# UCSD-Comp-Imaging/Nerf-Simple

Hardware: AMD Instinct MI355X
Metric: ray-samples/sec at 800x800x128 (higher is better)
Workload: dtype f16

## Files before the change

nerf-simple_amd/csrc/mlp_bf16_16.hip:

```cpp
#include "composite_device.h"
#include "launchers.h"

using namespace nerf_layout;

#ifdef NERF_HALF
typedef _Float16 elem_t;
#define NERF_MFMA __builtin_amdgcn_mfma_f32_16x16x32_f16
#define NERF_KERNEL nerf_mlp_f16_16_kernel
#define NERF_LAUNCH nerf_amd_launch_mlp_f16_16
#else
typedef __bf16 elem_t;
#define NERF_MFMA __builtin_amdgcn_mfma_f32_16x16x32_bf16
#define NERF_KERNEL nerf_mlp_bf16_16_kernel
#define NERF_LAUNCH nerf_amd_launch_mlp_bf16_16
#endif
#include "mlp16_chain.h"

namespace {

#ifdef NERF_HALF
constexpr bool FOLD = true;
#else
constexpr bool FOLD = false;
#endif
struct MlpPlan {
    static constexpr int LAYERS = NUM_LAYERS;
    static constexpr bool SAVE = !FOLD;
    static constexpr int tpc(int L) { return L == 0 ? 8 : 4; }
    static constexpr int mt(int L) { return FOLD ? fold_mt(L) : b16_mt(L); }
    static constexpr int layer_off_kib(int L) { return FOLD ? fold_layer_off_kib(L) : b16_layer_off_kib(L); }
    static constexpr int bias_off(int L) { return FOLD ? fold_bias_off(L) : b16_bias_off(L); }
};
static_assert(NUM_CHUNKS<MlpPlan> == (FOLD ? 34 : 38) && plan_fits<MlpPlan>(), "chunks per tile / weight buffer, parity");

constexpr int LDS_POSD = LDS_CHAIN_END;
constexpr int LDS_POSX = LDS_POSD + WAVES * NCB * 1024;
constexpr int LDS_TOTAL = LDS_POSX + WAVES * NCB * 2048;
constexpr int RING_PTS = 1024;
constexpr int LDS_RING_RAW = LDS_TOTAL;
constexpr int LDS_RING_T = LDS_RING_RAW + RING_PTS * 16;
constexpr int LDS_TOTAL_COMP = LDS_RING_T + RING_PTS * 4;
constexpr int COMP_MAX_N = RING_PTS - TILE_PTS;
static_assert(COMP_MAX_N == FUSED_RENDER_MAX_N, "api.hip routes by this limit");
static_assert(LDS_TOTAL_COMP <= 160 * 1024, "LDS budget");
static_assert((RING_PTS & (RING_PTS - 1)) == 0 && RING_PTS % TILE_PTS == 0, "ring indexing");

static_assert(ACT_TILE_PTS == TILE_PTS && MASK_TILE_PTS == TILE_PTS, "activation blocks and mask tiles are the kernel's tiles");

struct State {
    using Plan = MlpPlan;
    ex8 X[NCB][8], Y[NCB][8];
    f32x4 pend[NCB][2];
    float sigma[NCB], rgb[NCB][3];
    bool bad;
    unsigned posd_off[NCB];
    char* acts;
    long long P;
    long long tile;
    int loff[NCB];
    unsigned mb[NCB][2];
    float amax[4];
    long long mask_tile;
    long long p_end;
    unsigned ring_q0;
    WFrag* wf;
};

template <bool RAYS, int SAVE, bool COMP>
__device__ __forceinline__ void stage_inputs(const Ctx& c, const MlpArgs& a, long long tile_base, State& st) {
    const int col = c.lane & 15, g = c.lane >> 4;
    float u_mine = 0.f;
    bool dev_rng = false;
    long long b0 = 0;
    int r0 = 0;
    if constexpr (RAYS) {
        b0 = tile_base / a.N;
        r0 = (int)(tile_base - b0 * a.N);
    }
    const long long p_end = COMP ? st.p_end : a.P;
    const int last_local = (int)(p_end - 1 - tile_base);
    constexpr bool RAY_POSD = RAYS && !SAVE;
    if constexpr (RAY_POSD) {
        const int top = last_local < TILE_PTS - 1 ? last_local : TILE_PTS - 1;
        const int nrays = (int)(split_point(b0, r0, top, a.N).b - b0) + 1;
        for (int idx = threadIdx.x; idx < nrays * 32; idx += WAVES * 64) {
            const int ray = idx >> 5, slot = idx & 31, gg = slot >> 3, sl = slot & 7;
            const float* rp = a.rays + (b0 + ray) * 6 + 3;
            const float dx = rp[0], dy = rp[1], dz = rp[2];
            const float nrm = norm3(dx, dy, dz);
            float val = 0.f;
            if (sl < 6) {
                const int cd = sl >> 1;
                const float dc = __fdiv_rn(cd == 0 ? dx : cd == 1 ? dy : dz, nrm);
                val = enc_lane(to_revolutions(dc), 2 * gg + (sl & 1));
            } else if (sl == 6 && gg < 3) {
                val = __fdiv_rn(gg == 0 ? dx : gg == 1 ? dy : dz, nrm);
            }
            lds_store<elem_t>(LDS_POSD + ray * 64 + slot * 2, 0, (elem_t)val);
        }
    }
    if constexpr (RAYS && NCB == 2) {
        dev_rng = (a.flags & NERF_FLAG_DEVICE_RNG) && !(a.flags & NERF_FLAG_TS_GIVEN);
        if (dev_rng) {
            int lm = c.wave * 32 + (c.lane & 31);
            if (lm > last_local) lm = last_local;
            u_mine = device_rng_uniform(a, split_point(b0, r0, lm, a.N));
        }
    }
#pragma unroll
    for (int cb = 0; cb < NCB; ++cb) {
        long long p = tile_base + c.wave * (16 * NCB) + cb * 16 + col;
        const bool valid = p < p_end;
        st.loff[cb] = valid ? block_lane_offset(g, c.wave * (16 * NCB) + cb * 16 + col) : LOFF_INVALID;
        if constexpr (SAVE == 2) {
            if (cb == 0)
                st.loff[0] = tile_base + c.wave * 32 + 16 * (c.lane >> 5) + col < p_end ? f8_lane_offset(c.lane, c.wave) : LOFF_INVALID;
        }
        if (!valid) p = p_end - 1;
        PointIn pt;
        st.posd_off[cb] = c.b_posd + cb * 1024;
        if constexpr (RAYS) {
            const float u_cb = (NCB == 2) ? __shfl(u_mine, cb * 16 + col) : 0.f;
            int lp = c.wave * (16 * NCB) + cb * 16 + col;
            if (lp > last_local) lp = last_local;
            if (SAVE && a.pts) {
                pt = fetch_point_pts(a, p);
            } else {
                const RaySample rs = split_point(b0, r0, lp, a.N);
                if constexpr (RAY_POSD) st.posd_off[cb] = LDS_POSD + (unsigned)(rs.b - b0) * 64 + g * 16;
                pt = fetch_point_rays<!RAY_POSD>(a, p, rs, u_cb, dev_rng);
                if constexpr (COMP) {
                    if (valid && g == 0)
                        lds_store<float>(((st.ring_q0 + c.wave * (16 * NCB) + cb * 16 + col) & (RING_PTS - 1)) * 4, LDS_RING_T, pt.t);
                }
                if (valid && g == 0 && a.ts_out) a.ts_out[p] = pt.t;
            }
        } else {
            pt = fetch_point_pts(a, p);
        }
        {
            const float xyz[3] = {pt.x, pt.y, pt.z};
            float v[16];
#pragma unroll
            for (int cd = 0; cd < 3; ++cd) {
                const TwoF q = to_revolutions(xyz[cd]);
#pragma unroll
                for (int jj = 0; jj < 5; ++jj) v[cd * 5 + jj] = enc_lane(q, 5 * g + jj);
            }
            v[15] = g == 0 ? pt.x : g == 1 ? pt.y : g == 2 ? pt.z : 0.f;
#pragma unroll
            for (int e = 0; e < 2; ++e) {
                u32x4 r;
#pragma unroll
                for (int i = 0; i < 4; ++i) r[i] = pack2<false>(v[8 * e + 2 * i], v[8 * e + 2 * i + 1]);
                lds_store<u32x4>(c.b_posx, cb * 2048 + e * 1024, r);
            }
        }
        if constexpr (!RAY_POSD) {
            const float dd[3] = {pt.d1, pt.d2, pt.d3};
            float v[8];
#pragma unroll
            for (int cd = 0; cd < 3; ++cd) {
                const TwoF q = to_revolutions(dd[cd]);
#pragma unroll
                for (int jj = 0; jj < 2; ++jj) v[cd * 2 + jj] = enc_lane(q, 2 * g + jj);
            }
            v[6] = g == 0 ? pt.d1 : g == 1 ? pt.d2 : g == 2 ? pt.d3 : 0.f;
            v[7] = 0.f;
            u32x4 r;
#pragma unroll
            for (int i = 0; i < 4; ++i) r[i] = pack2<false>(v[2 * i], v[2 * i + 1]);
            lds_store<u32x4>(c.b_posd, cb * 1024, r);
        }
    }
}

template <bool RAYS, int SAVE, bool COMP>
__device__ __forceinline__ void run_tile(const Ctx& c, const MlpArgs& a, long long tile_base, State& st) {
    stage_inputs<RAYS, SAVE, COMP>(c, a, tile_base, st);
    run_layer<0, SAVE>(c, st, st.X, st.X);
    run_layer<1, SAVE>(c, st, st.X, st.Y);
    run_layer<2, SAVE>(c, st, st.Y, st.X);
    run_layer<3, SAVE>(c, st, st.X, st.Y);
    run_layer<4, SAVE>(c, st, st.Y, st.X);
    run_layer<5, SAVE>(c, st, st.X, st.Y);
    run_layer<6, SAVE>(c, st, st.Y, st.X);
    run_layer<7, SAVE>(c, st, st.X, st.Y);
    ex8 (&c_in)[NCB][8] = FOLD ? st.Y : st.X;
    ex8 (&c_out)[NCB][8] = FOLD ? st.X : st.Y;
    run_layer<8, SAVE>(c, st, st.Y, st.X);
    run_layer<9, SAVE>(c, st, c_in, c_out);
    run_layer<10, SAVE>(c, st, c_out, c_in);
    epilogue_piece<10, 0>(0, st.pend, st.X, st);
    for (int cb_ = 1; cb_ < NCB; ++cb_) epilogue_piece<10, 0>(4 * cb_, st.pend, st.X, st);
}

__device__ __forceinline__ bool finite4(float x, float y, float z, float w) {
    return __builtin_fabsf(x) + __builtin_fabsf(y) + __builtin_fabsf(z) + __builtin_fabsf(w) < __builtin_inff();
}

struct RingSamples {
    unsigned q0;
    __device__ __forceinline__ float t(int i) const {
        return lds_load<float>(((q0 + (unsigned)i) & (RING_PTS - 1)) * 4, LDS_RING_T);
    }
    __device__ __forceinline__ f32x4 c(int i) const {
        return lds_load<f32x4>(((q0 + (unsigned)i) & (RING_PTS - 1)) * 16, LDS_RING_RAW);
    }
};

template <bool RAYS, int SAVE, bool COMP>
__device__ __forceinline__ void kernel_body(const MlpArgs& a, long long ntiles) {
    static_assert(!COMP || (RAYS && !SAVE), "the fused render is the rays-mode inference kernel");
    using P = MlpPlan;
    Ctx c;
    c.wave = __builtin_amdgcn_readfirstlane(threadIdx.x >> 6);
    c.lane = threadIdx.x & 63;
    const char* img = reinterpret_cast<const char*>(a.packed);
    c.wrsrc = __builtin_amdgcn_make_buffer_rsrc(const_cast<char*>(img), 0, (int)B16_IMAGE_BYTES, 0x00020000);
    c.wave_goff = c.wave * 1024;
    c.lane16 = c.lane * 16;
#pragma unroll
    for (int p = 0; p < 2; ++p) {
        c.b_wread[p] = LDS_W0 + p * LDS_WBUF + c.lane * 16;
        c.s_wdst[p] = LDS_W0 + p * LDS_WBUF + c.wave * 1024;
    }
    c.b_bias = (c.lane >> 4) * 16;
    c.b_posx = LDS_POSX + c.wave * (NCB * 2048) + c.lane * 16;
    c.b_posd = LDS_POSD + c.wave * (NCB * 1024) + c.lane * 16;

    {
        const float* bsrc = reinterpret_cast<const float*>(img + (long long)B16_WEIGHT_KIB * 1024);
        for (int i = threadIdx.x; i < B16_BIAS_FLOATS; i += WAVES * 64)
            lds_store<float>(i * 4, LDS_BIAS, bsrc[i]);
        Stage<P, NUM_CHUNKS<P> - 1>::issue(c);
    }
    asm volatile("s_waitcnt vmcnt(0)" ::: "memory");
    __syncthreads();
    WFrag wf;
    {
        constexpr int F0 = chunk_tiles<P>(0) * (layer_desc(0).chain_k / 32 + layer_desc(0).extra_slots / 32);
#pragma unroll
        for (int f = 0; f < 4 && f < F0; ++f) wf.a[f] = lds_load<ex8>(c.b_wread[0], f * 1024);
        wf.bias0 = lds_load<f32x4>(c.b_bias, LDS_BIAS + P::bias_off(0) * 4);
    }

    if constexpr (!COMP) {
        for (long long tile = blockIdx.x; tile < ntiles; tile += gridDim.x) {
            const long long tile_base = tile * TILE_PTS;
            asm volatile("" : "+s"(c.wave_goff));
            State st;
            st.wf = &wf;
            st.acts = reinterpret_cast<char*>(a.acts);
            st.P = a.P;
            st.mask_tile = SAVE == 2 ? f8_mask_offset_bytes(0, tile, 0, a.P) : mask_offset_bytes(0, tile, 0, a.P);
            st.tile = tile;
            st.bad = false;
            run_tile<RAYS, SAVE, false>(c, a, tile_base, st);
            bool bad = st.bad;
            if (c.lane < 16) {
#pragma unroll
                for (int cb = 0; cb < NCB; ++cb) {
                    const long long p = tile_base + c.wave * (16 * NCB) + cb * 16 + c.lane;
                    if (p < a.P) {
                        const f32x4 o = {st.rgb[cb][0], st.rgb[cb][1], st.rgb[cb][2], st.sigma[cb]};
                        *reinterpret_cast<f32x4*>(a.raw + p * 4) = o;
                        bad |= !finite4(o[0], o[1], o[2], o[3]);
                    }
                }
            }
            flag_nonfinite(c, bad);
        }
    } else {
        const long long B = a.P / a.N;
        const long long r_lo = (long long)blockIdx.x * B / gridDim.x, r_hi = ((long long)blockIdx.x + 1) * B / gridDim.x;
        const long long range_base = r_lo * a.N;
        const int n_pts = (int)((r_hi - r_lo) * a.N);
        const nerf_composite::RayOut out{a.rgb, a.disp, a.alpha, a.acc, a.w, a.pixels};
        int next_ray = 0, n_complete = 0;
        for (int q_tile = 0; q_tile < n_pts; q_tile += TILE_PTS) {
            const long long tile_base = range_base + q_tile;
            asm volatile("" : "+s"(c.wave_goff));
            State st;
            st.wf = &wf;
            st.acts = nullptr;
            st.P = a.P;
            st.mask_tile = 0;
            st.tile = 0;
            st.p_end = range_base + n_pts;
            st.ring_q0 = (unsigned)q_tile & (RING_PTS - 1);
            st.bad = false;
            run_tile<true, false, true>(c, a, tile_base, st);
            bool bad = st.bad;
            if (c.lane < 16) {
#pragma unroll
                for (int cb = 0; cb < NCB; ++cb) {
                    const int local = c.wave * (16 * NCB) + cb * 16 + c.lane;
                    if (q_tile + local < n_pts) {
                        const f32x4 o = {st.rgb[cb][0], st.rgb[cb][1], st.rgb[cb][2], st.sigma[cb]};
                        lds_store<f32x4>(((st.ring_q0 + local) & (RING_PTS - 1)) * 16, LDS_RING_RAW, o);
                        bad |= !finite4(o[0], o[1], o[2], o[3]);
                    }
                }
            }
            flag_nonfinite(c, bad);
            asm volatile("s_waitcnt lgkmcnt(0)" ::: "memory");
            __builtin_amdgcn_s_barrier();
            asm volatile("" ::: "memory");
            const int done_q = q_tile + TILE_PTS < n_pts ? q_tile + TILE_PTS : n_pts;
            while ((n_complete + 1) * a.N <= done_q) ++n_complete;
            if (n_complete - next_ray >= WAVES || done_q + TILE_PTS - next_ray * a.N > RING_PTS || done_q == n_pts) {
                for (int ray = next_ray + c.wave; ray < n_complete; ray += WAVES) {
                    const long long gray = r_lo + ray;
                    const float* d = a.rays + gray * 6 + 3;
                    const float dnorm = nerf_composite::unit_dir_norm(d[0], d[1], d[2], true);
                    const RingSamples src{(unsigned)(ray * a.N) & (RING_PTS - 1)};
                    nerf_composite::composite_ray(src, a.N, c.lane, dnorm, gray, out);
                }
                next_ray = n_complete;
                asm volatile("s_waitcnt lgkmcnt(0)" ::: "memory");
                __builtin_amdgcn_s_barrier();
                asm volatile("" ::: "memory");
            }
        }
    }
}

template <bool RAYS, bool SAVE, bool COMP>
__global__ __launch_bounds__(WAVES * 64, WAVES / 4) void NERF_KERNEL(MlpArgs a, long long ntiles) {
    extern __shared__ __attribute__((aligned(16))) char smem[];
    (void)smem;
    kernel_body<RAYS, SAVE ? 1 : 0, COMP>(a, ntiles);
}
#ifndef NERF_HALF
__global__ __launch_bounds__(WAVES * 64, WAVES / 4) void nerf_mlp_train_e4m3_kernel(MlpArgs a, long long ntiles) {
    extern __shared__ __attribute__((aligned(16))) char smem[];
    (void)smem;
    kernel_body<true, 2, false>(a, ntiles);
}
#endif

}

extern "C" int NERF_LAUNCH(const MlpArgs* args, int rays_mode, hipStream_t stream) {
    (void)hipGetLastError();
    MlpArgs a = *args;
    if (a.P <= 0) return 0;
    const long long ntiles = (a.P + TILE_PTS - 1) / TILE_PTS;
    const int cus = device_cus();
    const long long grid = ntiles < cus ? ntiles : cus;
    hipError_t e = hipSuccess;
    const bool comp = a.rgb || a.disp || a.acc || a.alpha || a.w || a.pixels;
    if (comp) {
        if (!rays_mode || a.acts || a.N > COMP_MAX_N || a.P / grid + a.N >= (1ll << 31)) return -2;
        auto kern = NERF_KERNEL<true, false, true>;
        e = allow_dynamic_lds(reinterpret_cast<const void*>(kern), LDS_TOTAL_COMP);
        if (e != hipSuccess) return (int)e;
        hipLaunchKernelGGL(kern, dim3((unsigned)grid), dim3(WAVES * 64), LDS_TOTAL_COMP, stream, a, ntiles);
        return (int)hipGetLastError();
    }
#ifdef NERF_HALF
    if (a.acts) return -2;
    auto kern = rays_mode ? NERF_KERNEL<true, false, false> : NERF_KERNEL<false, false, false>;
#else
    if (a.acts && !rays_mode) return -2;
    if ((a.flags & NERF_FLAG_STORE_E4M3) && !a.acts) return -2;
    auto kern = a.acts ? ((a.flags & NERF_FLAG_STORE_E4M3) ? nerf_mlp_train_e4m3_kernel : NERF_KERNEL<true, true, false>)
                       : (rays_mode ? NERF_KERNEL<true, false, false> : NERF_KERNEL<false, false, false>);
#endif
    e = allow_dynamic_lds(reinterpret_cast<const void*>(kern), LDS_TOTAL);
    if (e != hipSuccess) return (int)e;
    hipLaunchKernelGGL(kern, dim3((unsigned)grid), dim3(WAVES * 64), LDS_TOTAL, stream, a, ntiles);
    return (int)hipGetLastError();
}
```

nerf-simple_amd/csrc/nerf_device.h:

```cpp
#pragma once
#include <hip/hip_runtime.h>
#include <stdint.h>
#include <atomic>
#include "nerf_layout.h"

typedef __bf16 bf16x8 __attribute__((ext_vector_type(8)));
typedef __bf16 bf16x2 __attribute__((ext_vector_type(2)));
typedef short s16x2 __attribute__((ext_vector_type(2)));
typedef unsigned short u16x2 __attribute__((ext_vector_type(2)));
typedef float f32x2 __attribute__((ext_vector_type(2)));
typedef float f32x4 __attribute__((ext_vector_type(4)));
typedef float f32x16 __attribute__((ext_vector_type(16)));
typedef unsigned u32x4 __attribute__((ext_vector_type(4)));

#define NERF_FLAG_TS_GIVEN 1u
#define NERF_FLAG_DEVICE_RNG 2u
#define NERF_FLAG_SEED_IN_MEMORY 4u
#define NERF_FLAG_STORE_E4M3 8u

struct MlpArgs {
    const float* pts;
    const float* rays;
    const float* u;
    const float* tbins;
    const void* packed;
    float* raw;
    float* ts_out;
    void* acts;
    long long P;
    long long ray_id0;
    unsigned long long seed;
    int N;
    unsigned flags;
    float* rgb;
    float* disp;
    float* alpha;
    float* acc;
    float* w;
    float* pixels;
};

struct DensityArgs {
    const float* pts;
    long long stride;
    const void* packed;
    float* sigma;
    long long P;
    long long ny, nz;
    float lo[3], step[3];
};

constexpr int NERF_MAX_DEVICES = 64;
inline int device_cus() {
    static int cache[NERF_MAX_DEVICES] = {};
    int dev = 0;
    if (hipGetDevice(&dev) != hipSuccess || dev < 0 || dev >= NERF_MAX_DEVICES) return 256;
    if (cache[dev] == 0) {
        int cus = 256;
        if (hipDeviceGetAttribute(&cus, hipDeviceAttributeMultiprocessorCount, dev) != hipSuccess || cus <= 0) cus = 256;
        cache[dev] = cus;
    }
    return cache[dev];
}
inline hipError_t allow_dynamic_lds(const void* kernel, int bytes) {
    struct Slot { const void* kernel; int dev; };
    static Slot slots[128];
    static std::atomic<int> used{0};
    int dev = 0;
    if (hipGetDevice(&dev) != hipSuccess) dev = -1;
    const int n = used.load(std::memory_order_acquire);
    for (int i = 0; i < n && i < 128; ++i)
        if (slots[i].kernel == kernel && slots[i].dev == dev) return hipSuccess;
    const hipError_t e = hipFuncSetAttribute(kernel, hipFuncAttributeMaxDynamicSharedMemorySize, bytes);
    if (e == hipSuccess && dev >= 0) {
        const int i = used.load(std::memory_order_relaxed);
        if (i < 128) {
            slots[i] = Slot{kernel, dev};
            used.store(i + 1, std::memory_order_release);
        }
    }
    return e;
}

constexpr int LOFF_INVALID = 0x40000000;
__host__ __device__ constexpr int swapped_chunk(int g) { return (g & 1) * 2 + (g >> 1); }
__host__ __device__ constexpr int block_lane_offset(int g, int local) { return swapped_chunk(g) * 4096 + local * 16; }

template <int AUX = 0>
__device__ __forceinline__ void store_granule(__amdgpu_buffer_rsrc_t rs, int voffset, int soffset, u32x4 w) {
    const auto s0 = __builtin_amdgcn_permlane16_swap(w[0], w[2], false, false);
    const auto s1 = __builtin_amdgcn_permlane16_swap(w[1], w[3], false, false);
    const unsigned o0 = s0[0], o1 = s1[0], o2 = s0[1], o3 = s1[1];
    __builtin_amdgcn_raw_buffer_store_b128(u32x4{o0, o1, o2, o3}, rs, voffset, soffset, AUX);
    asm volatile("s_nop 1" ::"v"(o0), "v"(o1), "v"(o2), "v"(o3) : "memory");
}

template <bool ABS>
__device__ __forceinline__ float f8_absmax(float running, float v0, float v1) {
    float r;
    if constexpr (ABS) asm("v_max3_f32 %0, %1, |%2|, |%3|" : "=v"(r) : "v"(running), "v"(v0), "v"(v1));
    else asm("v_max3_f32 %0, %1, %2, %3" : "=v"(r) : "v"(running), "v"(v0), "v"(v1));
    return r;
}
__device__ __forceinline__ int f8_wave_max_exponent(float m) {
    int r;
    asm volatile("s_nop 1\n\t"
                 "v_max_f32_dpp %1, %1, %1 quad_perm:[1,0,3,2] row_mask:0xf bank_mask:0xf\n\ts_nop 1\n\t"
                 "v_max_f32_dpp %1, %1, %1 quad_perm:[2,3,0,1] row_mask:0xf bank_mask:0xf\n\ts_nop 1\n\t"
                 "v_max_f32_dpp %1, %1, %1 row_half_mirror row_mask:0xf bank_mask:0xf\n\ts_nop 1\n\t"
                 "v_max_f32_dpp %1, %1, %1 row_mirror row_mask:0xf bank_mask:0xf\n\ts_nop 1\n\t"
                 "v_max_f32_dpp %1, %1, %1 row_bcast:15 row_mask:0xa bank_mask:0xf\n\ts_nop 1\n\t"
                 "v_max_f32_dpp %1, %1, %1 row_bcast:31 row_mask:0xc bank_mask:0xf\n\ts_nop 1\n\t"
                 "v_readlane_b32 %0, %1, 63"
                 : "=s"(r), "+v"(m));
    return (r >> 23) & 0xff;
}
__device__ __forceinline__ unsigned f8_cvt4(unsigned lo, unsigned hi, float scale) {
    unsigned r;
    asm("v_cvt_scalef32_pk_fp8_bf16 %0, %1, %3\n\tv_cvt_scalef32_pk_fp8_bf16 %0, %2, %3 op_sel:[0,0,1]"
        : "=&v"(r) : "v"(lo), "v"(hi), "s"(scale));
    return r;
}
__host__ __device__ constexpr int f8_lane_offset(int lane, int wave) {
    return ((lane >> 4) & 1) * 4096 + (wave * 32 + 16 * (lane >> 5) + (lane & 15)) * 16;
}
template <int AUX = 0>
__device__ __forceinline__ void store_fragment_f8(__amdgpu_buffer_rsrc_t rs_data, int voff, int soff_data, u32x4 w0, u32x4 w1,
                                                  float scale) {
    const unsigned a0 = f8_cvt4(w0[0], w0[1], scale), b0 = f8_cvt4(w0[2], w0[3], scale);
    unsigned a1 = f8_cvt4(w1[0], w1[1], scale), b1 = f8_cvt4(w1[2], w1[3], scale);
    asm volatile("s_nop 1" : "+v"(a1), "+v"(b1));
    const auto x0 = __builtin_amdgcn_permlane32_swap(a0, a1, false, false);
    const auto x1 = __builtin_amdgcn_permlane32_swap(b0, b1, false, false);
    const auto y0 = __builtin_amdgcn_permlane16_swap(x0[0], x1[0], false, false);
    const auto y1 = __builtin_amdgcn_permlane16_swap(x0[1], x1[1], false, false);
    const unsigned o0 = y0[0], o1 = y0[1], o2 = y1[0], o3 = y1[1];
#if defined(F8_TIMING) && F8_TIMING == 2
    asm volatile("" ::"v"(o0), "v"(o1), "v"(o2), "v"(o3));
#else
    __builtin_amdgcn_raw_buffer_store_b128(u32x4{o0, o1, o2, o3}, rs_data, voff, soff_data,
#if defined(F8_TIMING) && F8_TIMING == 3
                                           0);
#else
                                           AUX);
#endif
    asm volatile("s_nop 1" ::"v"(o0), "v"(o1), "v"(o2), "v"(o3) : "memory");
#endif
}
constexpr int F8_GROUP = 4;
template <int AUX = 0>
__device__ __forceinline__ void store_group_f8(__amdgpu_buffer_rsrc_t rs_data, int voff, int soff_data,
                                               __amdgpu_buffer_rsrc_t rs_scale, int lane, int scale_byte,
                                               const u32x4 (&w0)[F8_GROUP], const u32x4 (&w1)[F8_GROUP], float amax) {
#if defined(F8_TIMING) && F8_TIMING == 1
    const int e = (__builtin_bit_cast(int, amax) >> 23) & 0xff;
#else
    const int e = f8_wave_max_exponent(amax);
#endif
    const int sb = e > 8 ? e - 7 : 1;
    const float scale = __builtin_bit_cast(float, sb << 23);
#pragma unroll
    for (int k = 0; k < F8_GROUP; ++k) store_fragment_f8<AUX>(rs_data, voff, soff_data + k * 8192, w0[k], w1[k], scale);
#if !(defined(F8_TIMING) && F8_TIMING == 2)
    __builtin_amdgcn_raw_buffer_store_b32((unsigned)sb * 0x01010101u, rs_scale, lane == 0 ? scale_byte : LOFF_INVALID, 0, 0);
#endif
}

template <int N>
__device__ __forceinline__ void chunk_barrier() {
    asm volatile("s_waitcnt vmcnt(%0)" ::"n"(N) : "memory");
    __builtin_amdgcn_s_barrier();
    asm volatile("" ::: "memory");
}

__device__ __forceinline__ void wave_lds_fence() {
    __builtin_amdgcn_s_waitcnt(0xc07f);
    __builtin_amdgcn_wave_barrier();
}

typedef __attribute__((address_space(3))) char lds_char;
typedef __attribute__((address_space(3))) void lds_void;
template <class T>
__device__ __forceinline__ T lds_load(unsigned base, int imm) {
    return *reinterpret_cast<const __attribute__((address_space(3))) T*>(reinterpret_cast<lds_char*>(0) + base + imm);
}
template <class T>
__device__ __forceinline__ void lds_store(unsigned base, int imm, const T& v) {
    *reinterpret_cast<__attribute__((address_space(3))) T*>(reinterpret_cast<lds_char*>(0) + base + imm) = v;
}

template <class C, int NEXT, int KIB, int OFF_KIB, int WAVES>
struct ChunkDma {
    static constexpr int PIECES = (KIB + WAVES - 1) / WAVES;
    static constexpr int SRC_OFF = OFF_KIB * 1024;
    static __device__ __forceinline__ void issue_piece(const C& c, int p) {
        __builtin_amdgcn_raw_ptr_buffer_load_lds(
            c.wrsrc, reinterpret_cast<lds_void*>(reinterpret_cast<lds_char*>(0) + c.s_wdst[NEXT & 1] + p * (WAVES * 1024)), 16,
            c.lane16, c.wave_goff + (SRC_OFF + p * WAVES * 1024), 0, 0);
    }
    static __device__ __forceinline__ void issue(const C& c) {
#pragma unroll
        for (int p = 0; p < PIECES; ++p) issue_piece(c, p);
    }
};

__device__ __forceinline__ unsigned philox_word(unsigned long long seed, unsigned long long ctr) {
    unsigned c0 = (unsigned)ctr, c1 = (unsigned)(ctr >> 32), c2 = 0x6e657266u, c3 = 0x616d6421u;
    unsigned k0 = (unsigned)seed, k1 = (unsigned)(seed >> 32);
#pragma unroll
    for (int r = 0; r < 10; ++r) {
        const unsigned long long p0 = 0xD2511F53ull * c0, p1 = 0xCD9E8D57ull * c2;
        const unsigned n0 = (unsigned)(p1 >> 32) ^ c1 ^ k0, n2 = (unsigned)(p0 >> 32) ^ c3 ^ k1;
        c1 = (unsigned)p1; c3 = (unsigned)p0; c0 = n0; c2 = n2;
        k0 += 0x9E3779B9u; k1 += 0xBB67AE85u;
    }
    return c0;
}
__device__ __forceinline__ float philox_uniform(unsigned long long seed, unsigned long long ctr) {
    return (float)(philox_word(seed, ctr) >> 8) * (1.0f / 16777216.0f);
}

__device__ __forceinline__ float mul_rn(float a, float b) {
#pragma clang fp contract(off)
    return a * b;
}
__device__ __forceinline__ float add_rn(float a, float b) {
#pragma clang fp contract(off)
    return a + b;
}
__device__ __forceinline__ float sub_rn(float a, float b) {
#pragma clang fp contract(off)
    return a - b;
}
__device__ __forceinline__ float sqrt_rn(float a) { return sqrtf(a); }

__device__ __forceinline__ float norm3(float x, float y, float z) {
    return sqrt_rn(__fmaf_rn(z, z, __fmaf_rn(y, y, mul_rn(x, x))));
}

struct PointIn {
    float x, y, z, d1, d2, d3, t;
};

struct RaySample { long long b; int i; };
__device__ __forceinline__ RaySample split_point(long long b0, int r0, int local, int N) {
    const unsigned tt = (unsigned)(r0 + local);
    unsigned q = (unsigned)((float)tt * __frcp_rn((float)N));
    if ((long long)q * N > (long long)tt) --q;
    if ((long long)(q + 1) * N <= (long long)tt) ++q;
    return RaySample{b0 + q, (int)(tt - q * (unsigned)N)};
}
__device__ __forceinline__ RaySample split_point(long long p, int N) {
    const long long b = p / N;
    return RaySample{b, (int)(p - b * N)};
}

__device__ __forceinline__ unsigned long long effective_seed(const MlpArgs& a) {
    if (!(a.flags & NERF_FLAG_SEED_IN_MEMORY)) return a.seed;
    const unsigned long long v = *reinterpret_cast<const unsigned long long*>(a.u);
    const unsigned lo = __builtin_amdgcn_readfirstlane((unsigned)v), hi = __builtin_amdgcn_readfirstlane((unsigned)(v >> 32));
    return a.seed + (((unsigned long long)hi << 32) | lo);
}

__device__ __forceinline__ float device_rng_uniform(const MlpArgs& a, RaySample rs) {
    unsigned long long seed = effective_seed(a);
    asm volatile("" : "+s"(seed));
    return philox_uniform(seed, (unsigned long long)((a.ray_id0 + rs.b) * a.N + rs.i));
}

template <bool DIR = true>
__device__ __forceinline__ PointIn fetch_point_rays(const MlpArgs& a, long long p, RaySample rs, float u_pre = 0.f,
                                                    bool have_u = false) {
    PointIn r;
    const long long b = rs.b;
    const int i = rs.i;
    const float* ray = a.rays + b * 6;
    const float ox = ray[0], oy = ray[1], oz = ray[2];
    const float dx = ray[3], dy = ray[4], dz = ray[5];
    float t;
    if (a.flags & NERF_FLAG_TS_GIVEN) {
        t = __builtin_nontemporal_load(a.u + p);
    } else {
        float u;
        if (a.flags & NERF_FLAG_DEVICE_RNG)
            u = have_u ? u_pre : philox_uniform(effective_seed(a), (unsigned long long)((a.ray_id0 + b) * a.N + i));
        else
            u = __builtin_nontemporal_load(a.u + p);
        const float bin_diff = sub_rn(a.tbins[1], a.tbins[0]);
        t = add_rn(mul_rn(bin_diff, u), a.tbins[i]);
    }
    r.t = t;
    r.x = add_rn(ox, mul_rn(dx, t));
    r.y = add_rn(oy, mul_rn(dy, t));
    r.z = add_rn(oz, mul_rn(dz, t));
    if constexpr (DIR) {
        const float nrm = norm3(dx, dy, dz);
        r.d1 = __fdiv_rn(dx, nrm);
        r.d2 = __fdiv_rn(dy, nrm);
        r.d3 = __fdiv_rn(dz, nrm);
    } else {
        r.d1 = r.d2 = r.d3 = 0.f;
    }
    return r;
}

__device__ __forceinline__ PointIn fetch_point_rays(const MlpArgs& a, long long p) {
    return fetch_point_rays(a, p, split_point(p, a.N));
}

__device__ __forceinline__ PointIn fetch_point_pts(const MlpArgs& a, long long p) {
    PointIn r;
    const float* v = a.pts + p * 6;
    r.x = v[0]; r.y = v[1]; r.z = v[2];
    r.d1 = v[3]; r.d2 = v[4]; r.d3 = v[5];
    r.t = 0.f;
    return r;
}

struct TwoF { float hi, lo; };
__device__ __forceinline__ TwoF to_revolutions(float x) {
    const float C_HI = 0.15915494f;
    const float C_LO = 6.4206382e-09f;
    x = __builtin_amdgcn_fmed3f(x, -0x1p100f, 0x1p100f);
    TwoF q;
    q.hi = mul_rn(x, C_HI);
    const float err = __fmaf_rn(x, C_HI, -q.hi);
    q.lo = __fmaf_rn(x, C_LO, err);
    return q;
}
__device__ __forceinline__ float enc_lane(TwoF q, int idx) {
    const float sc = __builtin_amdgcn_ldexpf(1.0f, idx >> 1);
    const float fr = __builtin_amdgcn_fractf(q.hi * sc) + q.lo * sc + ((idx & 1) ? 0.25f : 0.f);
    return __builtin_amdgcn_sinf(fr);
}
__device__ __forceinline__ void sincos_rev_fast(TwoF q, float scale, float& s, float& c) {
    const float f = __builtin_amdgcn_fractf(q.hi * scale) + q.lo * scale;
    s = __builtin_amdgcn_sinf(f);
    c = __builtin_amdgcn_cosf(f);
}
```

Baseline: 1.370 billion.

## Use tile-relative 32-bit indexing in fused composite path and cache ray norms in LDS

In the fused MLP+composite path, per-point sample decomposition now uses tile-local 32-bit indices with a float reciprocal division instead of 64-bit division. Pointers and RNG counters are precomputed per tile. Ray direction norms are computed once during input staging and kept in a new LDS slot array, so compositing no longer reloads ray directions from global memory. The per-tile barrier moves inside the composite branch so it only runs when rays are actually composited. This adds LDS use and relies on the float-reciprocal split being exact for the index range.

```diff
diff --git a/nerf-simple_amd/csrc/mlp_bf16_16.hip b/nerf-simple_amd/csrc/mlp_bf16_16.hip
--- a/nerf-simple_amd/csrc/mlp_bf16_16.hip
+++ b/nerf-simple_amd/csrc/mlp_bf16_16.hip
@@ -39,7 +39,10 @@
 constexpr int RING_PTS = 1024;
 constexpr int LDS_RING_RAW = LDS_TOTAL;
 constexpr int LDS_RING_T = LDS_RING_RAW + RING_PTS * 16;
-constexpr int LDS_TOTAL_COMP = LDS_RING_T + RING_PTS * 4;
+constexpr int DNORM_SLOTS = RING_PTS / 2;
+constexpr int LDS_DNORM = LDS_RING_T + RING_PTS * 4;
+constexpr int LDS_TOTAL_COMP = LDS_DNORM + DNORM_SLOTS * 4;
+static_assert((DNORM_SLOTS & (DNORM_SLOTS - 1)) == 0, "dnorm slot indexing");
 constexpr int COMP_MAX_N = RING_PTS - TILE_PTS;
 static_assert(COMP_MAX_N == FUSED_RENDER_MAX_N, "api.hip routes by this limit");
 static_assert(LDS_TOTAL_COMP <= 160 * 1024, "LDS budget");
@@ -61,7 +64,11 @@
     unsigned mb[NCB][2];
     float amax[4];
     long long mask_tile;
-    long long p_end;
+    int last_local;
+    int r0;
+    unsigned lb0;
+    const float* rays_tile;
+    unsigned long long ctr_tile;
     unsigned ring_q0;
     WFrag* wf;
 };
@@ -73,19 +80,24 @@
     bool dev_rng = false;
     long long b0 = 0;
     int r0 = 0;
-    if constexpr (RAYS) {
+    if constexpr (COMP) {
+        r0 = st.r0;
+    } else if constexpr (RAYS) {
         b0 = tile_base / a.N;
         r0 = (int)(tile_base - b0 * a.N);
     }
-    const long long p_end = COMP ? st.p_end : a.P;
-    const int last_local = (int)(p_end - 1 - tile_base);
+    const long long p_end = a.P;
+    const int last_local = COMP ? st.last_local : (int)(p_end - 1 - tile_base);
+    const float* const u_tile = a.u + tile_base;
     constexpr bool RAY_POSD = RAYS && !SAVE;
     if constexpr (RAY_POSD) {
         const int top = last_local < TILE_PTS - 1 ? last_local : TILE_PTS - 1;
-        const int nrays = (int)(split_point(b0, r0, top, a.N).b - b0) + 1;
+        int nrays;
+        if constexpr (COMP) nrays = (int)split_point_tile(r0, top, a.N).q + 1;
+        else nrays = (int)(split_point(b0, r0, top, a.N).b - b0) + 1;
         for (int idx = threadIdx.x; idx < nrays * 32; idx += WAVES * 64) {
             const int ray = idx >> 5, slot = idx & 31, gg = slot >> 3, sl = slot & 7;
-            const float* rp = a.rays + (b0 + ray) * 6 + 3;
+            const float* rp = COMP ? st.rays_tile + (unsigned)ray * 6u + 3 : a.rays + (b0 + ray) * 6 + 3;
             const float dx = rp[0], dy = rp[1], dz = rp[2];
             const float nrm = norm3(dx, dy, dz);
             float val = 0.f;
@@ -97,6 +109,11 @@
                 val = __fdiv_rn(gg == 0 ? dx : gg == 1 ? dy : dz, nrm);
             }
             lds_store<elem_t>(LDS_POSD + ray * 64 + slot * 2, 0, (elem_t)val);
+            if constexpr (COMP) {
+                if (slot == 31 && a.N >= 2)
+                    lds_store<float>(((st.lb0 + (unsigned)ray) & (DNORM_SLOTS - 1)) * 4, LDS_DNORM,
+                                     nerf_composite::unit_dir_norm(dx, dy, dz, true));
+            }
         }
     }
     if constexpr (RAYS && NCB == 2) {
@@ -104,13 +121,19 @@
         if (dev_rng) {
             int lm = c.wave * 32 + (c.lane & 31);
             if (lm > last_local) lm = last_local;
-            u_mine = device_rng_uniform(a, split_point(b0, r0, lm, a.N));
+            if constexpr (COMP) {
+                unsigned long long seed = effective_seed(a);
+                asm volatile("" : "+s"(seed));
+                u_mine = philox_uniform(seed, st.ctr_tile + (unsigned)lm);
+            } else {
+                u_mine = device_rng_uniform(a, split_point(b0, r0, lm, a.N));
+            }
         }
     }
 #pragma unroll
     for (int cb = 0; cb < NCB; ++cb) {
         long long p = tile_base + c.wave * (16 * NCB) + cb * 16 + col;
-        const bool valid = p < p_end;
+        const bool valid = COMP ? c.wave * (16 * NCB) + cb * 16 + col <= last_local : p < p_end;
         st.loff[cb] = valid ? block_lane_offset(g, c.wave * (16 * NCB) + cb * 16 + col) : LOFF_INVALID;
         if constexpr (SAVE == 2) {
             if (cb == 0)
@@ -123,16 +146,20 @@
             const float u_cb = (NCB == 2) ? __shfl(u_mine, cb * 16 + col) : 0.f;
             int lp = c.wave * (16 * NCB) + cb * 16 + col;
             if (lp > last_local) lp = last_local;
-            if (SAVE && a.pts) {
+            if constexpr (COMP) {
+                const TileSample rs = split_point_tile(r0, lp, a.N);
+                st.posd_off[cb] = LDS_POSD + rs.q * 64 + g * 16;
+                pt = fetch_point_tile(a, st.rays_tile, u_tile, (unsigned)lp, rs, u_cb);
+                if (valid && g == 0) {
+                    lds_store<float>(((st.ring_q0 + c.wave * (16 * NCB) + cb * 16 + col) & (RING_PTS - 1)) * 4, LDS_RING_T, pt.t);
+                    if (a.ts_out) (a.ts_out + tile_base)[(unsigned)lp] = pt.t;
+                }
+            } else if (SAVE && a.pts) {
                 pt = fetch_point_pts(a, p);
             } else {
                 const RaySample rs = split_point(b0, r0, lp, a.N);
                 if constexpr (RAY_POSD) st.posd_off[cb] = LDS_POSD + (unsigned)(rs.b - b0) * 64 + g * 16;
                 pt = fetch_point_rays<!RAY_POSD>(a, p, rs, u_cb, dev_rng);
-                if constexpr (COMP) {
-                    if (valid && g == 0)
-                        lds_store<float>(((st.ring_q0 + c.wave * (16 * NCB) + cb * 16 + col) & (RING_PTS - 1)) * 4, LDS_RING_T, pt.t);
-                }
                 if (valid && g == 0 && a.ts_out) a.ts_out[p] = pt.t;
             }
         } else {
@@ -277,6 +304,7 @@
         const long long range_base = r_lo * a.N;
         const int n_pts = (int)((r_hi - r_lo) * a.N);
         const nerf_composite::RayOut out{a.rgb, a.disp, a.alpha, a.acc, a.w, a.pixels};
+        const unsigned long long ctr_base = (unsigned long long)a.ray_id0 * (unsigned long long)a.N + (unsigned long long)range_base;
         int next_ray = 0, n_complete = 0;
         for (int q_tile = 0; q_tile < n_pts; q_tile += TILE_PTS) {
             const long long tile_base = range_base + q_tile;
@@ -287,7 +315,11 @@
             st.P = a.P;
             st.mask_tile = 0;
             st.tile = 0;
-            st.p_end = range_base + n_pts;
+            st.lb0 = (unsigned)q_tile / (unsigned)a.N;
+            st.r0 = (int)((unsigned)q_tile - st.lb0 * (unsigned)a.N);
+            st.rays_tile = a.rays + (r_lo + st.lb0) * 6;
+            st.ctr_tile = ctr_base + (unsigned)q_tile;
+            st.last_local = n_pts - 1 - q_tile;
             st.ring_q0 = (unsigned)q_tile & (RING_PTS - 1);
             st.bad = false;
             run_tile<true, false, true>(c, a, tile_base, st);
@@ -304,16 +336,21 @@
                 }
             }
             flag_nonfinite(c, bad);
-            asm volatile("s_waitcnt lgkmcnt(0)" ::: "memory");
-            __builtin_amdgcn_s_barrier();
-            asm volatile("" ::: "memory");
             const int done_q = q_tile + TILE_PTS < n_pts ? q_tile + TILE_PTS : n_pts;
             while ((n_complete + 1) * a.N <= done_q) ++n_complete;
             if (n_complete - next_ray >= WAVES || done_q + TILE_PTS - next_ray * a.N > RING_PTS || done_q == n_pts) {
+                asm volatile("s_waitcnt lgkmcnt(0)" ::: "memory");
+                __builtin_amdgcn_s_barrier();
+                asm volatile("" ::: "memory");
                 for (int ray = next_ray + c.wave; ray < n_complete; ray += WAVES) {
                     const long long gray = r_lo + ray;
-                    const float* d = a.rays + gray * 6 + 3;
-                    const float dnorm = nerf_composite::unit_dir_norm(d[0], d[1], d[2], true);
+                    float dnorm;
+                    if (a.N >= 2) {
+                        dnorm = lds_load<float>(((unsigned)ray & (DNORM_SLOTS - 1)) * 4, LDS_DNORM);
+                    } else {
+                        const float* d = a.rays + gray * 6 + 3;
+                        dnorm = nerf_composite::unit_dir_norm(d[0], d[1], d[2], true);
+                    }
                     const RingSamples src{(unsigned)(ray * a.N) & (RING_PTS - 1)};
                     nerf_composite::composite_ray(src, a.N, c.lane, dnorm, gray, out);
                 }
diff --git a/nerf-simple_amd/csrc/nerf_device.h b/nerf-simple_amd/csrc/nerf_device.h
--- a/nerf-simple_amd/csrc/nerf_device.h
+++ b/nerf-simple_amd/csrc/nerf_device.h
@@ -308,6 +308,34 @@
     return fetch_point_rays(a, p, split_point(p, a.N));
 }
 
+struct TileSample { unsigned q; int i; };
+__device__ __forceinline__ TileSample split_point_tile(int r0, int local, int N) {
+    const unsigned tt = (unsigned)(r0 + local);
+    const unsigned q = (unsigned)(((float)tt + 0.5f) * __frcp_rn((float)N));
+    return TileSample{q, (int)(tt - __umul24(q, (unsigned)N))};
+}
+__device__ __forceinline__ PointIn fetch_point_tile(const MlpArgs& a, const float* rays_tile, const float* u_tile, unsigned local,
+                                                    TileSample rs, float u_pre) {
+    PointIn r;
+    const float* ray = rays_tile + rs.q * 6u;
+    const float ox = ray[0], oy = ray[1], oz = ray[2];
+    const float dx = ray[3], dy = ray[4], dz = ray[5];
+    float t;
+    if (a.flags & NERF_FLAG_TS_GIVEN) {
+        t = __builtin_nontemporal_load(u_tile + local);
+    } else {
+        const float u = (a.flags & NERF_FLAG_DEVICE_RNG) ? u_pre : __builtin_nontemporal_load(u_tile + local);
+        const float bin_diff = sub_rn(a.tbins[1], a.tbins[0]);
+        t = add_rn(mul_rn(bin_diff, u), a.tbins[rs.i]);
+    }
+    r.t = t;
+    r.x = add_rn(ox, mul_rn(dx, t));
+    r.y = add_rn(oy, mul_rn(dy, t));
+    r.z = add_rn(oz, mul_rn(dz, t));
+    r.d1 = r.d2 = r.d3 = 0.f;
+    return r;
+}
+
 __device__ __forceinline__ PointIn fetch_point_pts(const MlpArgs& a, long long p) {
     PointIn r;
     const float* v = a.pts + p * 6;
```

Result: no change. 1.379 billion, median of 6 (+0.6%).
